# aokomoriuta/ConjugateGradient

Measured on AMD Instinct MI355X. Metric: CG iterations/sec (7-pt Poisson 512^3); SpMV achieved HBM GB/s in roofline, higher is better.
Workload: dtype f64

## Files before the change

### conjugategradient_amd/csrc/kernels_block.hip

```cpp
#include "common.hpp"

namespace mgcg {

typedef double d2 __attribute__((ext_vector_type(2)));

struct BlockScalars {
    double rr[kBlockMaxK], rr0[kBlockMaxK], alpha[kBlockMaxK], beta[kBlockMaxK], residual[kBlockMaxK];
    int iteration[kBlockMaxK], status[kBlockMaxK], active[kBlockMaxK], mode[kBlockMaxK];
    int done, pad;
};

bool Workspace::ensure_block()
{
    if (blockPartials && blockScalars) return true;
    if (!blockPartials && !MGCG_HIP(hipMalloc((void**)&blockPartials, sizeof(double) * 3 * kBlockMaxK * (size_t)kMaxPartials))) return false;
    if (!blockScalars) {
        if (!MGCG_HIP(hipMalloc((void**)&blockScalars, sizeof(BlockScalars)))) return false;
        if (!MGCG_HIP(hipMemset(blockScalars, 0, sizeof(BlockScalars)))) return false;
    }
    return true;
}

template <int K, bool NT = false>
__device__ __forceinline__ void load_row(const double* p, double (&v)[K])
{
    if constexpr (K % 2 == 0) {
#pragma unroll
        for (int j = 0; j < K / 2; ++j) {
            d2 t;
            if constexpr (NT) t = __builtin_nontemporal_load((const d2*)p + j); else t = ((const d2*)p)[j];
            v[2 * j] = t.x; v[2 * j + 1] = t.y;
        }
    } else {
#pragma unroll
        for (int j = 0; j < K; ++j) { if constexpr (NT) v[j] = __builtin_nontemporal_load(p + j); else v[j] = p[j]; }
    }
}
template <int K, bool NT = false>
__device__ __forceinline__ void store_row(double* p, const double (&v)[K])
{
    if constexpr (K % 2 == 0) {
#pragma unroll
        for (int j = 0; j < K / 2; ++j) {
            d2 t; t.x = v[2 * j]; t.y = v[2 * j + 1];
            if constexpr (NT) __builtin_nontemporal_store(t, (d2*)p + j); else ((d2*)p)[j] = t;
        }
    } else {
#pragma unroll
        for (int j = 0; j < K; ++j) { if constexpr (NT) __builtin_nontemporal_store(v[j], p + j); else p[j] = v[j]; }
    }
}

__device__ __forceinline__ double wave_sum(double v)
{
#pragma unroll
    for (int off = 32; off > 0; off >>= 1) v += __shfl_down(v, off, 64);
    return v;
}
__device__ __forceinline__ double wave_max(double v)
{
#pragma unroll
    for (int off = 32; off > 0; off >>= 1) { double o = __shfl_down(v, off, 64); v = o > v ? o : v; }
    return v;
}
__device__ double block_reduce(const double* __restrict__ partials, int n, double* s_red, int mode)
{
    double acc = 0.0;
    if (mode == 0) { for (int i = threadIdx.x; i < n; i += kBlock) acc += partials[i]; acc = wave_sum(acc); }
    else { for (int i = threadIdx.x; i < n; i += kBlock) { double a = partials[i]; acc = a > acc ? a : acc; } acc = wave_max(acc); }
    __syncthreads();
    if ((threadIdx.x & 63) == 0) s_red[threadIdx.x >> 6] = acc;
    __syncthreads();
    if (mode == 0) return (s_red[0] + s_red[1]) + (s_red[2] + s_red[3]);
    double a = s_red[0] > s_red[1] ? s_red[0] : s_red[1];
    double b = s_red[2] > s_red[3] ? s_red[2] : s_red[3];
    return a > b ? a : b;
}

constexpr int kBTW = 4;
constexpr int kBTRows = 64 * kBTW;
constexpr int kBTCap = 512;
constexpr int kBNG = 8;

enum { BEPI_AP = 0,
       BEPI_RESIDUAL = 1,
       BEPI_PLAIN = 2 };

struct BlockSpmvArgs {
    const double* elements; const int* rowOffsets; const int* columnIndeces;
    const double* x;
    double* y;
    const double* b;
    long long ld;
    int rows;
    double* partials;
    const int* done;
};

template <int K, int EPI>
__device__ __forceinline__ void gather(const BlockSpmvArgs& a, int col, double (&v)[K])
{
    if constexpr (EPI == BEPI_AP) load_row<K>(a.x + (long long)col * K, v);
    else {
#pragma unroll
        for (int j = 0; j < K; ++j) v[j] = a.x[j * a.ld + col];
    }
}

template <int K, int EPI, bool NT>
__global__ __launch_bounds__(64 * kBTW) void spmv_block_kernel(BlockSpmvArgs a)
{
    __shared__ __attribute__((aligned(16))) int s_colAll[kBTCap * kBTW];
    __shared__ __attribute__((aligned(16))) double s_valAll[kBTCap * kBTW];
    if (a.done != nullptr && *a.done != 0) return;
    const int lane = threadIdx.x & 63, wv = threadIdx.x >> 6;
    int* s_col = s_colAll + wv * kBTCap;
    double* s_val = s_valAll + wv * kBTCap;
    const int nTiles = (a.rows + kBTRows - 1) / kBTRows;
    double dot[K];
#pragma unroll
    for (int j = 0; j < K; ++j) dot[j] = 0.0;
    for (int tile = blockIdx.x; tile < nTiles; tile += gridDim.x) {
        const int r0 = tile * kBTRows + wv * 64;
        const int row = r0 + lane;
        const bool valid = row < a.rows;
        const int rb = r0 < a.rows ? r0 : a.rows;
        const int rl = r0 + 64 < a.rows ? r0 + 64 : a.rows;
        const int s = a.rowOffsets[rb];
        const int e = a.rowOffsets[rl > rb ? rl : rb];
        const int rs = valid ? a.rowOffsets[row] : 0;
        const int re = valid ? a.rowOffsets[row + 1] : 0;
        const int cnt = re - rs;
        const bool staged = e - s <= kBTCap;
        if (staged) {
            for (int q = lane; q < e - s; q += 64) {
                if constexpr (NT) { s_col[q] = __builtin_nontemporal_load(a.columnIndeces + s + q); s_val[q] = __builtin_nontemporal_load(a.elements + s + q); }
                else { s_col[q] = a.columnIndeces[s + q]; s_val[q] = a.elements[s + q]; }
            }
        }
        __syncthreads();
        const bool fast = staged && __ballot(cnt > kBNG) == 0ull;
        double acc[K];
#pragma unroll
        for (int j = 0; j < K; ++j) acc[j] = 0.0;
        if (fast) {
            int cc[kBNG]; double vv[kBNG];
#pragma unroll
            for (int q = 0; q < kBNG; ++q) {
                const bool in = q < cnt;
                const int idx = in ? rs - s + q : 0;
                const int c = s_col[idx]; const double v = s_val[idx];
                cc[q] = in ? c : 0; vv[q] = in ? v : 0.0;
            }
            double xg[kBNG][K];
#pragma unroll
            for (int q = 0; q < kBNG; ++q) gather<K, EPI>(a, cc[q], xg[q]);
#pragma unroll
            for (int q = 0; q < kBNG; ++q) {
#pragma unroll
                for (int j = 0; j < K; ++j) { const double t = vv[q] * xg[q][j]; acc[j] += (q < cnt) ? t : 0.0; }
            }
        } else if (valid) {
            for (int q = rs; q < re; ++q) {
                int col; double v;
                if (staged) { col = s_col[q - s]; v = s_val[q - s]; }
                else if constexpr (NT) { col = __builtin_nontemporal_load(a.columnIndeces + q); v = __builtin_nontemporal_load(a.elements + q); }
                else { col = a.columnIndeces[q]; v = a.elements[q]; }
                double xv[K];
                gather<K, EPI>(a, col, xv);
#pragma unroll
                for (int j = 0; j < K; ++j) { const double t = v * xv[j]; acc[j] += t; }
            }
        }
        if (valid) {
            if constexpr (EPI == BEPI_AP) {
                double w[K];
                load_row<K>(a.x + (long long)row * K, w);
#pragma unroll
                for (int j = 0; j < K; ++j) { const double t = w[j] * acc[j]; dot[j] += t; }
                store_row<K, NT>(a.y + (long long)row * K, acc);
            } else if constexpr (EPI == BEPI_RESIDUAL) {
#pragma unroll
                for (int j = 0; j < K; ++j) a.y[j * a.ld + row] = a.b[j * a.ld + row] - acc[j];
            } else {
#pragma unroll
                for (int j = 0; j < K; ++j) a.y[j * a.ld + row] = acc[j];
            }
        }
        __syncthreads();
    }
    if constexpr (EPI == BEPI_AP) {
#pragma unroll
        for (int j = 0; j < K; ++j) {
            const double t = wave_sum(dot[j]);
            if (lane == 0) a.partials[(long long)j * kMaxPartials + blockIdx.x * kBTW + wv] = t;
        }
    }
}

template <int K>
static int launch_spmv_block(hipStream_t s, int epi, const BlockSpmvArgs& a, bool nt)
{
    if (a.rows <= 0) return 0;
    const int nTiles = (a.rows + kBTRows - 1) / kBTRows;
    DeviceState* d = device_state();
    int nWG = 2 * (d ? d->numCu : kNumCu);
    if (nWG > nTiles) nWG = nTiles;
    if (nWG * kBTW > kMaxPartials) nWG = kMaxPartials / kBTW;
#define GO(E, N) hipLaunchKernelGGL((spmv_block_kernel<K, E, N>), dim3(nWG), dim3(64 * kBTW), 0, s, a)
    if (epi == BEPI_AP) { if (nt) GO(BEPI_AP, true); else GO(BEPI_AP, false); }
    else if (epi == BEPI_RESIDUAL) { if (nt) GO(BEPI_RESIDUAL, true); else GO(BEPI_RESIDUAL, false); }
    else { if (nt) GO(BEPI_PLAIN, true); else GO(BEPI_PLAIN, false); }
#undef GO
    return nWG * kBTW;
}

static int vec_grid(long long n)
{
    long long g = (n + kBlock - 1) / kBlock;
    if (g > kMaxGrid) g = kMaxGrid;
    return g < 1 ? 1 : (int)g;
}

template <int K, bool INF>
__device__ __forceinline__ void block_partials_out(double (&acc)[K], double (&mx)[K], double* partials, double* partialsInf)
{
    __shared__ double s_sum[K][4];
    __shared__ double s_max[K][4];
#pragma unroll
    for (int j = 0; j < K; ++j) {
        const double t = wave_sum(acc[j]);
        if ((threadIdx.x & 63) == 0) s_sum[j][threadIdx.x >> 6] = t;
        if constexpr (INF) { const double m = wave_max(mx[j]); if ((threadIdx.x & 63) == 0) s_max[j][threadIdx.x >> 6] = m; }
    }
    __syncthreads();
    if (threadIdx.x < K) {
        const int j = threadIdx.x;
        partials[(long long)j * kMaxPartials + blockIdx.x] = (s_sum[j][0] + s_sum[j][1]) + (s_sum[j][2] + s_sum[j][3]);
        if constexpr (INF) {
            double a = s_max[j][0] > s_max[j][1] ? s_max[j][0] : s_max[j][1];
            double b = s_max[j][2] > s_max[j][3] ? s_max[j][2] : s_max[j][3];
            partialsInf[(long long)j * kMaxPartials + blockIdx.x] = a > b ? a : b;
        }
    }
}

template <int K>
__global__ __launch_bounds__(kBlock) void block_copy_dot_kernel(double* __restrict__ p, const double* __restrict__ r, long long n, double* __restrict__ partials)
{
    double acc[K], mx[K];
#pragma unroll
    for (int j = 0; j < K; ++j) { acc[j] = 0.0; mx[j] = 0.0; }
    for (long long i = (long long)blockIdx.x * kBlock + threadIdx.x; i < n; i += (long long)gridDim.x * kBlock) {
        double pv[K];
#pragma unroll
        for (int j = 0; j < K; ++j) { const double rv = r[j * n + i]; pv[j] = rv; const double t = rv * rv; acc[j] += t; }
        store_row<K>(p + i * K, pv);
    }
    block_partials_out<K, false>(acc, mx, partials, nullptr);
}

template <int K, bool INF, bool NT>
__global__ __launch_bounds__(kBlock) void block_update_r_kernel(const BlockScalars* __restrict__ sc, double* __restrict__ r, const double* __restrict__ Ap, long long n,
                                                                double* __restrict__ partials, double* __restrict__ partialsInf)
{
    if (sc->done != 0) return;
    bool act[K]; double malpha[K], acc[K], mx[K];
#pragma unroll
    for (int j = 0; j < K; ++j) { act[j] = sc->active[j] != 0; malpha[j] = -sc->alpha[j]; acc[j] = 0.0; mx[j] = 0.0; }
    for (long long i = (long long)blockIdx.x * kBlock + threadIdx.x; i < n; i += (long long)gridDim.x * kBlock) {
        double av[K];
        load_row<K, NT>(Ap + i * K, av);
#pragma unroll
        for (int j = 0; j < K; ++j) {
            if (!act[j]) continue;
            const double u = malpha[j] * av[j]; const double rv = r[j * n + i] + u; r[j * n + i] = rv;
            const double q = rv * rv; acc[j] += q;
            if constexpr (INF) { const double a0 = fabs(rv); mx[j] = a0 > mx[j] ? a0 : mx[j]; }
        }
    }
    block_partials_out<K, INF>(acc, mx, partials, partialsInf);
}

template <int K, bool NT>
__global__ __launch_bounds__(kBlock) void block_update_xp_kernel(const BlockScalars* __restrict__ sc, double* __restrict__ x, double* __restrict__ p,
                                                                 const double* __restrict__ r, long long n)
{
    int mode[K]; double al[K], be[K];
    bool any = false, anyP = false;
#pragma unroll
    for (int j = 0; j < K; ++j) { mode[j] = sc->mode[j]; al[j] = sc->alpha[j]; be[j] = sc->beta[j]; any = any || mode[j] > 0; anyP = anyP || mode[j] == 2; }
    if (!any) return;
    for (long long i = (long long)blockIdx.x * kBlock + threadIdx.x; i < n; i += (long long)gridDim.x * kBlock) {
        double pv[K];
        load_row<K, NT>(p + i * K, pv);
#pragma unroll
        for (int j = 0; j < K; ++j) {
            if (mode[j] == 0) continue;
            const double t = al[j] * pv[j]; x[j * n + i] = x[j * n + i] + t;
            if (mode[j] == 2) { const double u = be[j] * pv[j]; pv[j] = r[j * n + i] + u; }
        }
        if (anyP) store_row<K, NT>(p + i * K, pv);
    }
}

constexpr int kBSerialBatch = 2048;
__global__ __launch_bounds__(kBlock) void block_dot_serial_kernel(const double* __restrict__ x, const double* __restrict__ y, long long n,
                                                                  long long colStep, long long elemStep, double* __restrict__ out, const BlockScalars* sc)
{
    __shared__ double s_prod[2][kBSerialBatch];
    const int col = blockIdx.x;
    if (sc != nullptr && (sc->done != 0 || sc->active[col] == 0)) return;
    const double* xc = x + col * colStep;
    const double* yc = y + col * colStep;
    const int tid = threadIdx.x;
    const long long nBatches = (n + kBSerialBatch - 1) / kBSerialBatch;
    auto fill = [&](int buf, long long b) {
        const long long base = b * kBSerialBatch;
        for (int k = tid - kWave; k < kBSerialBatch; k += kBlock - kWave) {
            const long long i = base + k;
            double t = 0.0;
            if (i < n) t = xc[i * elemStep] * yc[i * elemStep];
            s_prod[buf][k] = t;
        }
    };
    if (tid >= kWave) fill(0, 0);
    __syncthreads();
    double acc = 0.0;
    for (long long b = 0; b < nBatches; ++b) {
        if (tid >= kWave) { if (b + 1 < nBatches) fill((int)((b + 1) & 1), b + 1); }
        else if (tid == 0) {
            const double* q = s_prod[b & 1];
#pragma unroll 16
            for (int k = 0; k < kBSerialBatch; ++k) acc += q[k];
        }
        __syncthreads();
    }
    if (tid == 0) out[(long long)col * kMaxPartials] = acc;
}

__global__ __launch_bounds__(kBlock) void block_init_kernel(BlockScalars* sc, const double* __restrict__ partials, int n, int k)
{
    __shared__ double s_red[4];
    for (int j = 0; j < kBlockMaxK; ++j) {
        const double rr = j < k ? block_reduce(partials + (long long)j * kMaxPartials, n, s_red, 0) : 0.0;
        if (threadIdx.x == 0) {
            sc->rr[j] = rr; sc->rr0[j] = rr; sc->alpha[j] = 0.0; sc->beta[j] = 0.0; sc->residual[j] = 0.0;
            sc->iteration[j] = 0; sc->status[j] = MGCG_OK; sc->active[j] = j < k ? 1 : 0; sc->mode[j] = 0;
        }
    }
    if (threadIdx.x == 0) { sc->done = k > 0 ? 0 : 1; sc->pad = 0; }
}

__global__ __launch_bounds__(kBlock) void block_alpha_kernel(BlockScalars* sc, const double* __restrict__ partials, int n, int k)
{
    __shared__ double s_red[4];
    if (sc->done != 0) return;
    for (int j = 0; j < k; ++j) {
        if (sc->active[j] == 0) continue;
        const double pAp = block_reduce(partials + (long long)j * kMaxPartials, n, s_red, 0);
        if (threadIdx.x == 0) sc->alpha[j] = sc->rr[j] / pAp;
    }
}

__global__ __launch_bounds__(kBlock) void block_finalize_kernel(BlockScalars* sc, const double* __restrict__ partials, int n,
                                                                const double* __restrict__ partialsInf, int nInf, int k, FinalizeArgs f)
{
    __shared__ double s_red[4];
    if (sc->done != 0) { if (threadIdx.x < kBlockMaxK) sc->mode[threadIdx.x] = 0; return; }
    for (int j = 0; j < k; ++j) {
        if (sc->active[j] == 0) { if (threadIdx.x == 0) sc->mode[j] = 0; continue; }
        const double rrNew = block_reduce(partials + (long long)j * kMaxPartials, n, s_red, 0);
        const double inf = partialsInf != nullptr ? block_reduce(partialsInf + (long long)j * kMaxPartials, nInf, s_red, 1) : 0.0;
        if (threadIdx.x == 0) {
            const int it = sc->iteration[j];
            const StopDecision d = decide_stop(f, rrNew, inf, sc->rr0[j], it);
            if (f.trace != nullptr && it < f.traceCap) f.trace[(long long)j * f.traceCap + it] = d.shown;
            sc->residual[j] = d.res;
            if (d.stop) { sc->mode[j] = 1; sc->active[j] = 0; sc->status[j] = d.status; }
            else { sc->mode[j] = 2; sc->beta[j] = rrNew / sc->rr[j]; sc->rr[j] = rrNew; sc->iteration[j] = it + 1; }
        }
    }
    if (threadIdx.x == 0) {
        int any = 0;
        for (int j = 0; j < k; ++j) any |= sc->active[j];
        sc->done = any ? 0 : 1;
    }
}

__global__ void block_snapshot_kernel(const BlockScalars* sc, volatile int* slot) { *slot = sc->done; }

struct BlockRun {
    Workspace* ws;
    const double* elements; const int* rowOffsets; const int* columnIndeces; int nnz;
    long long n;
    double *x; const double* b; double *Ap, *p, *r;
    double tol; int minIt, maxIt, rule;
};

template <int K>
static bool block_enqueue_init(const BlockRun& R, bool nt)
{
    hipStream_t s = R.ws->stream;
    double* P0 = R.ws->blockPartials;
    if (R.rule == MGCG_RULE_SIMPLE) launch_fill(s, R.x, 0.0, K * R.n);
    BlockSpmvArgs a{};
    a.elements = R.elements; a.rowOffsets = R.rowOffsets; a.columnIndeces = R.columnIndeces;
    a.x = R.x; a.y = R.r; a.b = R.b; a.ld = R.n; a.rows = (int)R.n;
    (void)launch_spmv_block<K>(s, BEPI_RESIDUAL, a, nt);
    const int g = vec_grid(R.n);
    hipLaunchKernelGGL((block_copy_dot_kernel<K>), dim3(g), dim3(kBlock), 0, s, R.p, R.r, R.n, P0);
    int nP = g;
    if (dot_reference_order()) {
        hipLaunchKernelGGL(block_dot_serial_kernel, dim3(K), dim3(kBlock), 0, s, R.r, R.r, R.n, R.n, 1LL, P0, (const BlockScalars*)nullptr);
        nP = 1;
    }
    hipLaunchKernelGGL(block_init_kernel, dim3(1), dim3(kBlock), 0, s, R.ws->blockScalars, P0, nP, K);
    return MGCG_HIP(hipGetLastError());
}

template <int K>
static bool block_enqueue_iteration(const BlockRun& R, bool nt, const FinalizeArgs& f)
{
    hipStream_t s = R.ws->stream;
    BlockScalars* sc = R.ws->blockScalars;
    double* P0 = R.ws->blockPartials;
    double* P1 = P0 + (size_t)kBlockMaxK * kMaxPartials;
    double* P2 = P1 + (size_t)kBlockMaxK * kMaxPartials;
    const bool ref = dot_reference_order();
    const bool inf = R.rule == MGCG_RULE_HANDMADECL;
    BlockSpmvArgs a{};
    a.elements = R.elements; a.rowOffsets = R.rowOffsets; a.columnIndeces = R.columnIndeces;
    a.x = R.p; a.y = R.Ap; a.ld = R.n; a.rows = (int)R.n; a.partials = P0; a.done = &sc->done;
    int nPAp = launch_spmv_block<K>(s, BEPI_AP, a, nt);
    if (ref) { hipLaunchKernelGGL(block_dot_serial_kernel, dim3(K), dim3(kBlock), 0, s, R.p, R.Ap, R.n, 1LL, (long long)K, P0, (const BlockScalars*)sc); nPAp = 1; }
    hipLaunchKernelGGL(block_alpha_kernel, dim3(1), dim3(kBlock), 0, s, sc, P0, nPAp, K);
    const int g = vec_grid(R.n);
#define GO(I, N) hipLaunchKernelGGL((block_update_r_kernel<K, I, N>), dim3(g), dim3(kBlock), 0, s, sc, R.r, R.Ap, R.n, P1, P2)
    if (inf) { if (nt) GO(true, true); else GO(true, false); }
    else { if (nt) GO(false, true); else GO(false, false); }
#undef GO
    int nRR = g;
    if (ref) { hipLaunchKernelGGL(block_dot_serial_kernel, dim3(K), dim3(kBlock), 0, s, R.r, R.r, R.n, R.n, 1LL, P1, (const BlockScalars*)sc); nRR = 1; }
    hipLaunchKernelGGL(block_finalize_kernel, dim3(1), dim3(kBlock), 0, s, sc, P1, nRR, inf ? P2 : nullptr, g, K, f);
    if (nt) hipLaunchKernelGGL((block_update_xp_kernel<K, true>), dim3(g), dim3(kBlock), 0, s, sc, R.x, R.p, R.r, R.n);
    else hipLaunchKernelGGL((block_update_xp_kernel<K, false>), dim3(g), dim3(kBlock), 0, s, sc, R.x, R.p, R.r, R.n);
    return MGCG_HIP(hipGetLastError());
}

template <int K>
static int block_solve(BlockRun& R, int iteration[], double residual[], int status[], double residualTrace[], int traceCapacity)
{
    Workspace* ws = R.ws;
    hipStream_t s = ws->stream;
    if (!ws->ensure_block()) return MGCG_ERROR;
    const int devTraceCap = (residualTrace && traceCapacity > 0) ? traceCapacity : 0;
    if (devTraceCap && !ws->ensure_trace(K * devTraceCap)) return MGCG_ERROR;
    const bool nt = R.n >= 8000000;
    FinalizeArgs f{};
    f.trace = devTraceCap ? ws->trace : nullptr; f.traceCap = devTraceCap;
    f.tol = R.tol; f.minIt = R.minIt; f.maxIt = R.maxIt; f.rule = R.rule;
    int checkEvery = 4;
    { const int v = tuning().checkEvery.load(std::memory_order_relaxed); if (v >= 1) checkEvery = v; }
    const long long hostCap = (long long)(R.maxIt > R.minIt ? R.maxIt : R.minIt) + 4;
    hipEvent_t ev[2] = { nullptr, nullptr };
    volatile int* slots = (volatile int*)&ws->hostScalar[2];
    bool ok = MGCG_HIP(hipEventCreateWithFlags(&ev[0], hipEventDisableTiming)) && MGCG_HIP(hipEventCreateWithFlags(&ev[1], hipEventDisableTiming));
    for (int i = 0; i < 4; ++i) slots[i] = 0;
    ok = ok && block_enqueue_init<K>(R, nt);
    long long enqueued = 0;
    int chunk = 0;
    bool finished = false;
    while (ok && !finished) {
        for (int i = 0; ok && i < checkEvery; ++i) ok = block_enqueue_iteration<K>(R, nt, f);
        enqueued += checkEvery;
        hipLaunchKernelGGL(block_snapshot_kernel, dim3(1), dim3(1), 0, s, (const BlockScalars*)ws->blockScalars, &slots[chunk & 1]);
        ok = ok && MGCG_HIP(hipEventRecord(ev[chunk & 1], s));
        if (chunk > 0) {
            ok = ok && MGCG_HIP(hipEventSynchronize(ev[(chunk - 1) & 1]));
            if (ok && slots[(chunk - 1) & 1] != 0) finished = true;
        }
        if (!finished && enqueued > hostCap + 2LL * checkEvery) {
            ok = ok && MGCG_HIP(hipStreamSynchronize(s));
            if (ok && slots[chunk & 1] != 0) finished = true;
            else { set_error("SolveBlockEx: the device never raised its stop flag after %lld iterations", enqueued); ok = false; }
        }
        ++chunk;
    }
    ok = MGCG_HIP(hipStreamSynchronize(s)) && ok;
    int worst = MGCG_OK;
    if (ok) {
        BlockScalars h;
        ok = MGCG_HIP(hipMemcpy(&h, ws->blockScalars, sizeof(BlockScalars), hipMemcpyDeviceToHost));
        for (int j = 0; ok && j < K; ++j) {
            if (iteration) iteration[j] = h.iteration[j];
            if (residual) residual[j] = h.residual[j];
            if (status) status[j] = h.status[j];
            if (h.status[j] == MGCG_NONFINITE) worst = MGCG_NONFINITE;
            else if (h.status[j] == MGCG_MAXIT_EXCEEDED && worst == MGCG_OK) worst = MGCG_MAXIT_EXCEEDED;
            if (devTraceCap) {
                int nTrace = h.iteration[j] + 1; if (nTrace > devTraceCap) nTrace = devTraceCap;
                ok = MGCG_HIP(hipMemcpy(residualTrace + (size_t)j * traceCapacity, ws->trace + (size_t)j * devTraceCap, sizeof(double) * (size_t)nTrace, hipMemcpyDeviceToHost));
            }
        }
        if (ok && worst == MGCG_NONFINITE) set_error("SolveBlockEx: the residual of a column is not finite");
        else if (ok && worst == MGCG_MAXIT_EXCEEDED) set_error("SolveBlockEx: a column did not converge within maxIteration %d", R.maxIt);
    }
    if (ev[0]) (void)hipEventDestroy(ev[0]);
    if (ev[1]) (void)hipEventDestroy(ev[1]);
    return ok ? worst : MGCG_ERROR;
}

template <int K>
static void csrmv_block(hipStream_t s, double* y, const double* elements, const int* rowOffsets, const int* columnIndeces, const double* x, int count)
{
    BlockSpmvArgs a{};
    a.elements = elements; a.rowOffsets = rowOffsets; a.columnIndeces = columnIndeces;
    a.x = x; a.y = y; a.ld = count; a.rows = count;
    (void)launch_spmv_block<K>(s, BEPI_PLAIN, a, count >= 8000000);
}

void preload_kernels_block() { preload_code_object(reinterpret_cast<const void*>(&block_snapshot_kernel)); }

}

using namespace mgcg;

extern "C" {

int SolveBlockEx(MgcgBlas* cublas, MgcgSparse* cusparse, MgcgMatDescr* matDescr,
                 Vector* elementsVector, VectorInt* rowOffsetsVector, VectorInt* columnIndecesVector,
                 Vector* xVector, Vector* bVector, Vector* ApVector, Vector* pVector, Vector* rVector,
                 int elementsCount, int count, int k,
                 double allowableResidual, int minIteration, int maxIteration, int rule,
                 int iteration[], double residual[], int status[], double residualTrace[], int traceCapacity)
{
    (void)matDescr;
    if (!device_state()) return MGCG_ERROR;
    if (!cublas || !cusparse) { set_error("SolveBlockEx: null handle"); return MGCG_ERROR; }
    if (k < 1 || k > kBlockMaxK) { set_error("SolveBlockEx: k = %d right-hand sides, must be 1 .. %d", k, kBlockMaxK); return MGCG_ERROR; }
    if (rule < MGCG_RULE_NATIVE || rule > MGCG_RULE_VIENNACL) { set_error("SolveBlockEx: unknown stop rule %d", rule); return MGCG_ERROR; }
    Vector* vs[6] = { elementsVector, xVector, bVector, ApVector, pVector, rVector };
    for (Vector* v : vs) if (!v) { set_error("SolveBlockEx: null vector handle"); return MGCG_ERROR; }
    if (!rowOffsetsVector || !columnIndecesVector) { set_error("SolveBlockEx: null vector handle"); return MGCG_ERROR; }
    if (elementsCount < 0 || count < 1) { set_error("SolveBlockEx: bad sizes"); return MGCG_ERROR; }
    const long long kn = (long long)k * count;
    if (elementsVector->size < elementsCount || columnIndecesVector->size < elementsCount || rowOffsetsVector->size < (long long)count + 1 ||
        xVector->size < kn || bVector->size < kn || ApVector->size < kn || pVector->size < kn || rVector->size < kn) {
        set_error("SolveBlockEx: a device vector is smaller than the problem (x, b, Ap, p, r need k * count entries)"); return MGCG_ERROR;
    }
    if (residualTrace && traceCapacity > 0 && (long long)k * traceCapacity > 0x7fffffffLL) { set_error("SolveBlockEx: trace capacity too large"); return MGCG_ERROR; }
    BlockRun R{};
    R.ws = &cublas->ws;
    R.elements = elementsVector->data; R.rowOffsets = rowOffsetsVector->data; R.columnIndeces = columnIndecesVector->data; R.nnz = elementsCount;
    R.n = count;
    R.x = xVector->data; R.b = bVector->data; R.Ap = ApVector->data; R.p = pVector->data; R.r = rVector->data;
    R.tol = allowableResidual; R.minIt = minIteration; R.maxIt = maxIteration; R.rule = rule;
    analysis_note_write(R.x, sizeof(double) * (size_t)kn);
    analysis_note_write(R.r, sizeof(double) * (size_t)kn);
    analysis_note_write(R.p, sizeof(double) * (size_t)kn);
    analysis_note_write(R.Ap, sizeof(double) * (size_t)kn);
    switch (k) {
    case 1: return block_solve<1>(R, iteration, residual, status, residualTrace, traceCapacity);
    case 2: return block_solve<2>(R, iteration, residual, status, residualTrace, traceCapacity);
    case 3: return block_solve<3>(R, iteration, residual, status, residualTrace, traceCapacity);
    case 4: return block_solve<4>(R, iteration, residual, status, residualTrace, traceCapacity);
    case 5: return block_solve<5>(R, iteration, residual, status, residualTrace, traceCapacity);
    case 6: return block_solve<6>(R, iteration, residual, status, residualTrace, traceCapacity);
    case 7: return block_solve<7>(R, iteration, residual, status, residualTrace, traceCapacity);
    default: return block_solve<8>(R, iteration, residual, status, residualTrace, traceCapacity);
    }
}

void CsrMVBlock(MgcgSparse* cusparse, MgcgMatDescr* matDescr, double* y, const double* elements, const int* rowOffsets,
                const int* columnIndeces, const double* x, int elementsCount, int count, int k)
{
    (void)matDescr;
    if (!device_state()) return;
    if (!cusparse || !y || !rowOffsets || !x || (elementsCount > 0 && (!elements || !columnIndeces))) { set_error("CsrMVBlock: null argument"); return; }
    if (k < 1 || k > kBlockMaxK) { set_error("CsrMVBlock: k = %d columns, must be 1 .. %d", k, kBlockMaxK); return; }
    if (count < 0 || elementsCount < 0) { set_error("CsrMVBlock: negative size"); return; }
    if (count == 0) return;
    analysis_note_write(y, sizeof(double) * (size_t)k * (size_t)count);
    hipStream_t s = cusparse->ws.stream;
    switch (k) {
    case 1: csrmv_block<1>(s, y, elements, rowOffsets, columnIndeces, x, count); break;
    case 2: csrmv_block<2>(s, y, elements, rowOffsets, columnIndeces, x, count); break;
    case 3: csrmv_block<3>(s, y, elements, rowOffsets, columnIndeces, x, count); break;
    case 4: csrmv_block<4>(s, y, elements, rowOffsets, columnIndeces, x, count); break;
    case 5: csrmv_block<5>(s, y, elements, rowOffsets, columnIndeces, x, count); break;
    case 6: csrmv_block<6>(s, y, elements, rowOffsets, columnIndeces, x, count); break;
    case 7: csrmv_block<7>(s, y, elements, rowOffsets, columnIndeces, x, count); break;
    default: csrmv_block<8>(s, y, elements, rowOffsets, columnIndeces, x, count); break;
    }
    (void)MGCG_HIP(hipGetLastError());
}

}
```

Baseline: 276.3.

## Add software-pipelined block SpMV kernel with tile map, 7-wide gather and NT tuning

Adds a pipelined block SpMV kernel that prefetches the next tile's row offsets and vectorized matrix slab into registers while the current tile's gathers run. It delays the output store by one trip. It also walks tiles through a shared tile map driven by the detected matrix period, and picks a 7-entry gather width when the maximum row length allows. Nontemporal policy is chosen by a row-count window. The intent is to hide load latency and trim padded gathers, at the cost of more registers, clamped overfetch and a period analysis on the host.

```diff
diff --git a/conjugategradient_amd/csrc/kernels_block.hip b/conjugategradient_amd/csrc/kernels_block.hip
--- a/conjugategradient_amd/csrc/kernels_block.hip
+++ b/conjugategradient_amd/csrc/kernels_block.hip
@@ -1,4 +1,5 @@
 #include "common.hpp"
+#include "spmv_epilogue.hpp"
 
 namespace mgcg {
 
@@ -80,7 +81,9 @@
 constexpr int kBTW = 4;
 constexpr int kBTRows = 64 * kBTW;
 constexpr int kBTCap = 512;
-constexpr int kBNG = 8;
+static_assert(kBTRows == kRowTileRows, "the block kernels walk the row-tile kernel's tiles (make_tile_map, MgcgDebugTileOrder)");
+
+typedef int i4 __attribute__((ext_vector_type(4)));
 
 enum { BEPI_AP = 0,
        BEPI_RESIDUAL = 1,
@@ -93,6 +96,7 @@
     const double* b;
     long long ld;
     int rows;
+    int nnz;
     double* partials;
     const int* done;
 };
@@ -107,20 +111,64 @@
     }
 }
 
-template <int K, int EPI, bool NT>
-__global__ __launch_bounds__(64 * kBTW) void spmv_block_kernel(BlockSpmvArgs a)
-{
+template <int K, int EPI>
+__device__ __forceinline__ void own_row(const BlockSpmvArgs& a, int row, double (&w)[K])
+{
+    if constexpr (EPI == BEPI_AP) load_row<K>(a.x + (long long)row * K, w);
+    else if constexpr (EPI == BEPI_RESIDUAL) {
+#pragma unroll
+        for (int j = 0; j < K; ++j) w[j] = a.b[j * a.ld + row];
+    } else {
+#pragma unroll
+        for (int j = 0; j < K; ++j) w[j] = 0.0;
+    }
+}
+template <int K, int EPI>
+__device__ __forceinline__ void row_value(const double (&w)[K], double (&acc)[K], double (&dot)[K])
+{
+#pragma unroll
+    for (int j = 0; j < K; ++j) {
+        if constexpr (EPI == BEPI_AP) { const double t = w[j] * acc[j]; dot[j] += t; }
+        else if constexpr (EPI == BEPI_RESIDUAL) acc[j] = w[j] - acc[j];
+    }
+}
+template <int K, int EPI, bool NTS>
+__device__ __forceinline__ void store_out(const BlockSpmvArgs& a, int row, const double (&v)[K])
+{
+    if constexpr (EPI == BEPI_AP) store_row<K, NTS>(a.y + (long long)row * K, v);
+    else {
+#pragma unroll
+        for (int j = 0; j < K; ++j) a.y[j * a.ld + row] = v[j];
+    }
+}
+template <int K, int EPI>
+__device__ __forceinline__ void write_partials(const BlockSpmvArgs& a, const double (&dot)[K], int lane, int wv)
+{
+    if constexpr (EPI == BEPI_AP) {
+#pragma unroll
+        for (int j = 0; j < K; ++j) {
+            const double t = wave_sum(dot[j]);
+            if (lane == 0) a.partials[(long long)j * kMaxPartials + blockIdx.x * kBTW + wv] = t;
+        }
+    }
+}
+
+template <int K, int EPI, int NG, int NT>
+__global__ __launch_bounds__(64 * kBTW) void spmv_block_kernel(BlockSpmvArgs a, TileMap tm, int nTiles)
+{
+    constexpr bool NTM = NT == 1, NTS = NT != 0;
     __shared__ __attribute__((aligned(16))) int s_colAll[kBTCap * kBTW];
     __shared__ __attribute__((aligned(16))) double s_valAll[kBTCap * kBTW];
     if (a.done != nullptr && *a.done != 0) return;
     const int lane = threadIdx.x & 63, wv = threadIdx.x >> 6;
     int* s_col = s_colAll + wv * kBTCap;
     double* s_val = s_valAll + wv * kBTCap;
-    const int nTiles = (a.rows + kBTRows - 1) / kBTRows;
     double dot[K];
 #pragma unroll
     for (int j = 0; j < K; ++j) dot[j] = 0.0;
-    for (int tile = blockIdx.x; tile < nTiles; tile += gridDim.x) {
+    const int nTrips = tile_map_trips(tm, blockIdx.x, gridDim.x, nTiles);
+    for (int t = 0; t < nTrips; ++t) {
+        const int tile = tile_map_tile(tm, t, blockIdx.x, gridDim.x);
         const int r0 = tile * kBTRows + wv * 64;
         const int row = r0 + lane;
         const bool valid = row < a.rows;
@@ -134,29 +182,29 @@
         const bool staged = e - s <= kBTCap;
         if (staged) {
             for (int q = lane; q < e - s; q += 64) {
-                if constexpr (NT) { s_col[q] = __builtin_nontemporal_load(a.columnIndeces + s + q); s_val[q] = __builtin_nontemporal_load(a.elements + s + q); }
+                if constexpr (NTM) { s_col[q] = __builtin_nontemporal_load(a.columnIndeces + s + q); s_val[q] = __builtin_nontemporal_load(a.elements + s + q); }
                 else { s_col[q] = a.columnIndeces[s + q]; s_val[q] = a.elements[s + q]; }
             }
         }
         __syncthreads();
-        const bool fast = staged && __ballot(cnt > kBNG) == 0ull;
+        const bool fast = staged && __ballot(cnt > NG) == 0ull;
         double acc[K];
 #pragma unroll
         for (int j = 0; j < K; ++j) acc[j] = 0.0;
         if (fast) {
-            int cc[kBNG]; double vv[kBNG];
-#pragma unroll
-            for (int q = 0; q < kBNG; ++q) {
+            int cc[NG]; double vv[NG];
+#pragma unroll
+            for (int q = 0; q < NG; ++q) {
                 const bool in = q < cnt;
                 const int idx = in ? rs - s + q : 0;
                 const int c = s_col[idx]; const double v = s_val[idx];
                 cc[q] = in ? c : 0; vv[q] = in ? v : 0.0;
             }
-            double xg[kBNG][K];
-#pragma unroll
-            for (int q = 0; q < kBNG; ++q) gather<K, EPI>(a, cc[q], xg[q]);
-#pragma unroll
-            for (int q = 0; q < kBNG; ++q) {
+            double xg[NG][K];
+#pragma unroll
+            for (int q = 0; q < NG; ++q) gather<K, EPI>(a, cc[q], xg[q]);
+#pragma unroll
+            for (int q = 0; q < NG; ++q) {
 #pragma unroll
                 for (int j = 0; j < K; ++j) { const double t = vv[q] * xg[q][j]; acc[j] += (q < cnt) ? t : 0.0; }
             }
@@ -164,7 +212,7 @@
             for (int q = rs; q < re; ++q) {
                 int col; double v;
                 if (staged) { col = s_col[q - s]; v = s_val[q - s]; }
-                else if constexpr (NT) { col = __builtin_nontemporal_load(a.columnIndeces + q); v = __builtin_nontemporal_load(a.elements + q); }
+                else if constexpr (NTM) { col = __builtin_nontemporal_load(a.columnIndeces + q); v = __builtin_nontemporal_load(a.elements + q); }
                 else { col = a.columnIndeces[q]; v = a.elements[q]; }
                 double xv[K];
                 gather<K, EPI>(a, col, xv);
@@ -173,33 +221,163 @@
             }
         }
         if (valid) {
-            if constexpr (EPI == BEPI_AP) {
-                double w[K];
-                load_row<K>(a.x + (long long)row * K, w);
-#pragma unroll
-                for (int j = 0; j < K; ++j) { const double t = w[j] * acc[j]; dot[j] += t; }
-                store_row<K, NT>(a.y + (long long)row * K, acc);
-            } else if constexpr (EPI == BEPI_RESIDUAL) {
-#pragma unroll
-                for (int j = 0; j < K; ++j) a.y[j * a.ld + row] = a.b[j * a.ld + row] - acc[j];
+            double w[K];
+            own_row<K, EPI>(a, row, w);
+            row_value<K, EPI>(w, acc, dot);
+            store_out<K, EPI, NTS>(a, row, acc);
+        }
+        __syncthreads();
+    }
+    write_partials<K, EPI>(a, dot, lane, wv);
+}
+
+template <int K, int EPI, int NG, int NT>
+__global__ __launch_bounds__(64 * kBTW) void spmv_block_pipe_kernel(BlockSpmvArgs a, TileMap tm, int nTiles)
+{
+    constexpr bool NTM = NT == 1, NTS = NT != 0;
+    __shared__ __attribute__((aligned(16))) int s_colAll[kBTCap * kBTW];
+    __shared__ __attribute__((aligned(16))) double s_valAll[kBTCap * kBTW];
+    if (a.done != nullptr && *a.done != 0) return;
+    const int lane = threadIdx.x & 63, wv = threadIdx.x >> 6;
+    int* s_col = s_colAll + wv * kBTCap;
+    double* s_val = s_valAll + wv * kBTCap;
+    const int wg = blockIdx.x, nWG = gridDim.x;
+    const int kMax4 = (a.nnz - 4) & ~3;
+    const int kMax2 = (a.nnz - 2) & ~1;
+    const int nTrips = tile_map_trips(tm, wg, nWG, nTiles);
+    double dot[K];
+#pragma unroll
+    for (int j = 0; j < K; ++j) dot[j] = 0.0;
+    if (nTrips > 0) {
+        auto tile_of = [&](int t) -> int {
+            t = t < nTrips ? t : nTrips - 1;
+            return tile_map_tile(tm, t, wg, nWG);
+        };
+        int roA_s, roA_e, roB_s, roB_e;
+        i4 c0, c1; d2 v0, v1, v2, v3;
+        auto load_ro = [&](int tile, int& rs, int& re) {
+            const int r = tile * kBTRows + wv * 64 + lane;
+            rs = a.rowOffsets[r]; re = a.rowOffsets[r + 1];
+        };
+        auto load_raw = [&](int s) {
+            const int tb = s & ~3;
+            int k0 = tb + 4 * lane, k1 = k0 + 256;
+            k0 = k0 < kMax4 ? k0 : kMax4; k1 = k1 < kMax4 ? k1 : kMax4;
+            int j0 = tb + 2 * lane, j1 = j0 + 128, j2 = j0 + 256, j3 = j0 + 384;
+            j0 = j0 < kMax2 ? j0 : kMax2; j1 = j1 < kMax2 ? j1 : kMax2; j2 = j2 < kMax2 ? j2 : kMax2; j3 = j3 < kMax2 ? j3 : kMax2;
+            if constexpr (NTM) {
+                c0 = __builtin_nontemporal_load((const i4*)(a.columnIndeces + k0)); c1 = __builtin_nontemporal_load((const i4*)(a.columnIndeces + k1));
+                v0 = __builtin_nontemporal_load((const d2*)(a.elements + j0)); v1 = __builtin_nontemporal_load((const d2*)(a.elements + j1));
+                v2 = __builtin_nontemporal_load((const d2*)(a.elements + j2)); v3 = __builtin_nontemporal_load((const d2*)(a.elements + j3));
             } else {
-#pragma unroll
-                for (int j = 0; j < K; ++j) a.y[j * a.ld + row] = acc[j];
+                c0 = *(const i4*)(a.columnIndeces + k0); c1 = *(const i4*)(a.columnIndeces + k1);
+                v0 = *(const d2*)(a.elements + j0); v1 = *(const d2*)(a.elements + j1); v2 = *(const d2*)(a.elements + j2); v3 = *(const d2*)(a.elements + j3);
             }
-        }
-        __syncthreads();
-    }
-    if constexpr (EPI == BEPI_AP) {
-#pragma unroll
-        for (int j = 0; j < K; ++j) {
-            const double t = wave_sum(dot[j]);
-            if (lane == 0) a.partials[(long long)j * kMaxPartials + blockIdx.x * kBTW + wv] = t;
-        }
-    }
+        };
+        int tileCur = tile_of(0), tileNext = tile_of(1);
+        load_ro(tileCur, roA_s, roA_e);
+        __builtin_amdgcn_sched_barrier(0);
+        load_raw(__builtin_amdgcn_readfirstlane(roA_s));
+        __builtin_amdgcn_sched_barrier(0);
+        load_ro(tileNext, roB_s, roB_e);
+        __builtin_amdgcn_sched_barrier(0);
+        double pend[K];
+#pragma unroll
+        for (int j = 0; j < K; ++j) pend[j] = 0.0;
+        int pendRow = tileCur * kBTRows + wv * 64 + lane;
+        for (int t = 0; t < nTrips; ++t) {
+            const int s = __builtin_amdgcn_readfirstlane(roA_s);
+            const int e = __builtin_amdgcn_readlane(roA_e, 63);
+            const int tb = s & ~3;
+            const int my_s = roA_s, my_e = roA_e, cnt = roA_e - roA_s;
+            const int row = tileCur * kBTRows + wv * 64 + lane;
+            const bool spanOk = (e - tb <= kBTCap) && (e <= kMax4 + 4);
+            const bool fast = spanOk && __ballot(cnt > NG) == 0ull;
+            *(i4*)(s_col + 4 * lane) = c0; *(i4*)(s_col + 256 + 4 * lane) = c1;
+            *(d2*)(s_val + 2 * lane) = v0; *(d2*)(s_val + 128 + 2 * lane) = v1; *(d2*)(s_val + 256 + 2 * lane) = v2; *(d2*)(s_val + 384 + 2 * lane) = v3;
+            __syncthreads();
+            int cc[NG]; double vv[NG];
+            double accSlow[K];
+#pragma unroll
+            for (int j = 0; j < K; ++j) accSlow[j] = 0.0;
+            if (fast) {
+#pragma unroll
+                for (int q = 0; q < NG; ++q) {
+                    int idx = my_s - tb + q;
+                    idx = q < cnt ? idx : 0;
+                    cc[q] = s_col[idx]; vv[q] = s_val[idx];
+                }
+            } else {
+#pragma unroll
+                for (int q = 0; q < NG; ++q) { cc[q] = 0; vv[q] = 0.0; }
+                for (int q = my_s; q < my_e; ++q) {
+                    const int col = a.columnIndeces[q];
+                    const double v = a.elements[q];
+                    double xv[K];
+                    gather<K, EPI>(a, col, xv);
+#pragma unroll
+                    for (int j = 0; j < K; ++j) { const double p = v * xv[j]; accSlow[j] += p; }
+                }
+            }
+            __builtin_amdgcn_sched_barrier(0);
+            double xg[NG][K];
+#pragma unroll
+            for (int q = 0; q < NG; ++q) gather<K, EPI>(a, cc[q], xg[q]);
+            double w[K];
+            own_row<K, EPI>(a, row, w);
+            store_out<K, EPI, NTS>(a, pendRow, pend);
+            load_raw(__builtin_amdgcn_readfirstlane(roB_s));
+            roA_s = roB_s; roA_e = roB_e;
+            const int tileAfter = tile_of(t + 2);
+            load_ro(tileAfter, roB_s, roB_e);
+            __builtin_amdgcn_sched_barrier(0);
+            double acc[K];
+#pragma unroll
+            for (int j = 0; j < K; ++j) acc[j] = 0.0;
+#pragma unroll
+            for (int q = 0; q < NG; ++q) {
+#pragma unroll
+                for (int j = 0; j < K; ++j) { const double p = vv[q] * xg[q][j]; acc[j] += (q < cnt) ? p : 0.0; }
+            }
+#pragma unroll
+            for (int j = 0; j < K; ++j) acc[j] = fast ? acc[j] : accSlow[j];
+            row_value<K, EPI>(w, acc, dot);
+#pragma unroll
+            for (int j = 0; j < K; ++j) pend[j] = acc[j];
+            pendRow = row;
+            __syncthreads();
+            tileCur = tileNext; tileNext = tileAfter;
+        }
+        store_out<K, EPI, NTS>(a, pendRow, pend);
+    }
+    write_partials<K, EPI>(a, dot, lane, wv);
+}
+
+constexpr int kBPipeMaxK = 8;
+
+template <int K, int EPI, int NT>
+static void launch_block_epi(hipStream_t s, const BlockSpmvArgs& a, const TileMap& tm, int nWG, int nTiles, bool seven, bool pipe)
+{
+    const dim3 g(nWG), b(64 * kBTW);
+    if constexpr (K <= kBPipeMaxK) {
+        if (pipe) {
+            if (seven) hipLaunchKernelGGL((spmv_block_pipe_kernel<K, EPI, 7, NT>), g, b, 0, s, a, tm, nTiles);
+            else hipLaunchKernelGGL((spmv_block_pipe_kernel<K, EPI, 8, NT>), g, b, 0, s, a, tm, nTiles);
+            return;
+        }
+    }
+    if (seven) hipLaunchKernelGGL((spmv_block_kernel<K, EPI, 7, NT>), g, b, 0, s, a, tm, nTiles);
+    else hipLaunchKernelGGL((spmv_block_kernel<K, EPI, 8, NT>), g, b, 0, s, a, tm, nTiles);
+}
+
+static int block_spmv_nt(long long rows, bool ntVectors)
+{
+    if (rows >= 8000000 && rows <= 36000000) return 1;
+    return ntVectors ? 2 : 0;
 }
 
 template <int K>
-static int launch_spmv_block(hipStream_t s, int epi, const BlockSpmvArgs& a, bool nt)
+static int launch_spmv_block(hipStream_t s, int epi, const BlockSpmvArgs& a, int periodRows, int maxRow, int nt)
 {
     if (a.rows <= 0) return 0;
     const int nTiles = (a.rows + kBTRows - 1) / kBTRows;
@@ -207,10 +385,15 @@
     int nWG = 2 * (d ? d->numCu : kNumCu);
     if (nWG > nTiles) nWG = nTiles;
     if (nWG * kBTW > kMaxPartials) nWG = kMaxPartials / kBTW;
-#define GO(E, N) hipLaunchKernelGGL((spmv_block_kernel<K, E, N>), dim3(nWG), dim3(64 * kBTW), 0, s, a)
-    if (epi == BEPI_AP) { if (nt) GO(BEPI_AP, true); else GO(BEPI_AP, false); }
-    else if (epi == BEPI_RESIDUAL) { if (nt) GO(BEPI_RESIDUAL, true); else GO(BEPI_RESIDUAL, false); }
-    else { if (nt) GO(BEPI_PLAIN, true); else GO(BEPI_PLAIN, false); }
+    const TileMap tm = make_tile_map(a.rows, periodRows, nWG, kBTRows);
+    const bool seven = maxRow > 0 && maxRow <= 7;
+    const bool pipe = tm.mode != 0 && a.nnz >= 8 && ((((uintptr_t)a.elements) | ((uintptr_t)a.columnIndeces)) & 15) == 0;
+#define GO(E) do { if (nt == 1) launch_block_epi<K, E, 1>(s, a, tm, nWG, nTiles, seven, pipe); \
+                   else if (nt == 2 && E == BEPI_AP) launch_block_epi<K, E, E == BEPI_AP ? 2 : 0>(s, a, tm, nWG, nTiles, seven, pipe); \
+                   else launch_block_epi<K, E, 0>(s, a, tm, nWG, nTiles, seven, pipe); } while (0)
+    if (epi == BEPI_AP) GO(BEPI_AP);
+    else if (epi == BEPI_RESIDUAL) GO(BEPI_RESIDUAL);
+    else GO(BEPI_PLAIN);
 #undef GO
     return nWG * kBTW;
 }
@@ -396,6 +579,7 @@
     long long n;
     double *x; const double* b; double *Ap, *p, *r;
     double tol; int minIt, maxIt, rule;
+    int periodRows, maxRow;
 };
 
 template <int K>
@@ -406,8 +590,8 @@
     if (R.rule == MGCG_RULE_SIMPLE) launch_fill(s, R.x, 0.0, K * R.n);
     BlockSpmvArgs a{};
     a.elements = R.elements; a.rowOffsets = R.rowOffsets; a.columnIndeces = R.columnIndeces;
-    a.x = R.x; a.y = R.r; a.b = R.b; a.ld = R.n; a.rows = (int)R.n;
-    (void)launch_spmv_block<K>(s, BEPI_RESIDUAL, a, nt);
+    a.x = R.x; a.y = R.r; a.b = R.b; a.ld = R.n; a.rows = (int)R.n; a.nnz = R.nnz;
+    (void)launch_spmv_block<K>(s, BEPI_RESIDUAL, a, R.periodRows, R.maxRow, block_spmv_nt(R.n, nt));
     const int g = vec_grid(R.n);
     hipLaunchKernelGGL((block_copy_dot_kernel<K>), dim3(g), dim3(kBlock), 0, s, R.p, R.r, R.n, P0);
     int nP = g;
@@ -431,8 +615,8 @@
     const bool inf = R.rule == MGCG_RULE_HANDMADECL;
     BlockSpmvArgs a{};
     a.elements = R.elements; a.rowOffsets = R.rowOffsets; a.columnIndeces = R.columnIndeces;
-    a.x = R.p; a.y = R.Ap; a.ld = R.n; a.rows = (int)R.n; a.partials = P0; a.done = &sc->done;
-    int nPAp = launch_spmv_block<K>(s, BEPI_AP, a, nt);
+    a.x = R.p; a.y = R.Ap; a.ld = R.n; a.rows = (int)R.n; a.nnz = R.nnz; a.partials = P0; a.done = &sc->done;
+    int nPAp = launch_spmv_block<K>(s, BEPI_AP, a, R.periodRows, R.maxRow, block_spmv_nt(R.n, nt));
     if (ref) { hipLaunchKernelGGL(block_dot_serial_kernel, dim3(K), dim3(kBlock), 0, s, R.p, R.Ap, R.n, 1LL, (long long)K, P0, (const BlockScalars*)sc); nPAp = 1; }
     hipLaunchKernelGGL(block_alpha_kernel, dim3(1), dim3(kBlock), 0, s, sc, P0, nPAp, K);
     const int g = vec_grid(R.n);
@@ -512,12 +696,14 @@
 }
 
 template <int K>
-static void csrmv_block(hipStream_t s, double* y, const double* elements, const int* rowOffsets, const int* columnIndeces, const double* x, int count)
+static void csrmv_block(MgcgSparse* h, double* y, const double* elements, const int* rowOffsets, const int* columnIndeces, const double* x, int elementsCount, int count)
 {
     BlockSpmvArgs a{};
     a.elements = elements; a.rowOffsets = rowOffsets; a.columnIndeces = columnIndeces;
-    a.x = x; a.y = y; a.ld = count; a.rows = count;
-    (void)launch_spmv_block<K>(s, BEPI_PLAIN, a, count >= 8000000);
+    a.x = x; a.y = y; a.ld = count; a.rows = count; a.nnz = elementsCount;
+    int maxRow = 0;
+    const int periodRows = elementsCount >= 8 ? spmv_period(h, rowOffsets, columnIndeces, count, 0, &maxRow) : 0;
+    (void)launch_spmv_block<K>(h->ws.stream, BEPI_PLAIN, a, periodRows, maxRow, block_spmv_nt(count, false));
 }
 
 void preload_kernels_block() { preload_code_object(reinterpret_cast<const void*>(&block_snapshot_kernel)); }
@@ -556,6 +742,7 @@
     R.n = count;
     R.x = xVector->data; R.b = bVector->data; R.Ap = ApVector->data; R.p = pVector->data; R.r = rVector->data;
     R.tol = allowableResidual; R.minIt = minIteration; R.maxIt = maxIteration; R.rule = rule;
+    if (elementsCount >= 8) R.periodRows = spmv_period(cusparse, R.rowOffsets, R.columnIndeces, R.n, 0, &R.maxRow);
     analysis_note_write(R.x, sizeof(double) * (size_t)kn);
     analysis_note_write(R.r, sizeof(double) * (size_t)kn);
     analysis_note_write(R.p, sizeof(double) * (size_t)kn);
@@ -582,16 +769,15 @@
     if (count < 0 || elementsCount < 0) { set_error("CsrMVBlock: negative size"); return; }
     if (count == 0) return;
     analysis_note_write(y, sizeof(double) * (size_t)k * (size_t)count);
-    hipStream_t s = cusparse->ws.stream;
     switch (k) {
-    case 1: csrmv_block<1>(s, y, elements, rowOffsets, columnIndeces, x, count); break;
-    case 2: csrmv_block<2>(s, y, elements, rowOffsets, columnIndeces, x, count); break;
-    case 3: csrmv_block<3>(s, y, elements, rowOffsets, columnIndeces, x, count); break;
-    case 4: csrmv_block<4>(s, y, elements, rowOffsets, columnIndeces, x, count); break;
-    case 5: csrmv_block<5>(s, y, elements, rowOffsets, columnIndeces, x, count); break;
-    case 6: csrmv_block<6>(s, y, elements, rowOffsets, columnIndeces, x, count); break;
-    case 7: csrmv_block<7>(s, y, elements, rowOffsets, columnIndeces, x, count); break;
-    default: csrmv_block<8>(s, y, elements, rowOffsets, columnIndeces, x, count); break;
+    case 1: csrmv_block<1>(cusparse, y, elements, rowOffsets, columnIndeces, x, elementsCount, count); break;
+    case 2: csrmv_block<2>(cusparse, y, elements, rowOffsets, columnIndeces, x, elementsCount, count); break;
+    case 3: csrmv_block<3>(cusparse, y, elements, rowOffsets, columnIndeces, x, elementsCount, count); break;
+    case 4: csrmv_block<4>(cusparse, y, elements, rowOffsets, columnIndeces, x, elementsCount, count); break;
+    case 5: csrmv_block<5>(cusparse, y, elements, rowOffsets, columnIndeces, x, elementsCount, count); break;
+    case 6: csrmv_block<6>(cusparse, y, elements, rowOffsets, columnIndeces, x, elementsCount, count); break;
+    case 7: csrmv_block<7>(cusparse, y, elements, rowOffsets, columnIndeces, x, elementsCount, count); break;
+    default: csrmv_block<8>(cusparse, y, elements, rowOffsets, columnIndeces, x, elementsCount, count); break;
     }
     (void)MGCG_HIP(hipGetLastError());
 }
```

After: 265.6. 0.961x the previous value.
